# LiXirong/pytorch-r2d2

Hardware: AMD Instinct MI355X
Metric: learner_steps_per_sec (higher is better)
Workload: dtype fp32; 1 GPU; model=r2d2-qnet (reference model.py: conv32x3 + LSTM256 + dueling, 6 actions), preset=atari57, global_batch=64, per_gpu_batch=64, seq_len=80, burn_in=40, n_step=5, target_mode=fixed, matmul=bf16x3 split (fp32 accumulate, fp32 state/storage), replay_rows_per_gpu=999936, parallelism=dp1, hip_graph=True, hoisted_step=True, graph_chunk=8

## Files before the change

csrc/kernels/torso.hip:

```cpp
#include "../common.h"

template <int CIN_, int H_, int W_>
struct TGeo {
  static constexpr int CIN = CIN_, H = H_, W = W_;
  static constexpr int IN_BYTES = CIN * H * W;
  static constexpr int IN_CHUNKS = IN_BYTES / 16;
  static constexpr int NT = 512;
  static constexpr int PF = (IN_CHUNKS + 319) / 320;
  static constexpr int H1 = (H - 8) / 4 + 1, W1 = (W - 8) / 4 + 1;
  static constexpr int H2 = (H1 - 4) / 2 + 1, W2 = (W1 - 4) / 2 + 1;
  static constexpr int H3 = H2 - 2, W3 = W2 - 2;
  static constexpr int P1 = H1 * W1, P2 = H2 * W2, P3 = H3 * W3;
  static constexpr int OUT = 32 * P3;
  static constexpr int H4 = H / 4, W4 = W / 4;
  static constexpr int K1S = 4 * CIN;
  static constexpr int ACTS = 40;
  static constexpr int W2S = 512 + 8;
  static constexpr int W3S = 288 + 8;
  static constexpr int S2DS = 16 * CIN + 8;
  static constexpr int OFF_IN = 0;
  static constexpr int OFF_A1 = OFF_IN + H4 * W4 * S2DS * 2;
  static constexpr int A1_BYTES = ((P1 + 3) / 4) * 256;
  static constexpr int OFF_A2 = OFF_A1 + A1_BYTES;
  static constexpr int OFF_W2 = OFF_A2 + P2 * ACTS * 2;
  static constexpr int OFF_W3 = OFF_W2 + 32 * W2S * 2;
  static constexpr int OFF_B23 = OFF_W3 + 32 * W3S * 2;
  static constexpr int LDS_BYTES = OFF_B23 + 64 * 4;
  static_assert(H % 4 == 0 && W % 4 == 0 && IN_BYTES % 16 == 0, "geometry");
  static_assert((P1 + 31) / 32 == 13 && (P2 + 31) / 32 == 3 && (P3 + 31) / 32 == 2, "tile deal");
  static_assert(OFF_A1 % 16 == 0 && LDS_BYTES <= 160 * 1024, "LDS");
};
using GeoAtari = TGeo<4, 84, 84>;
using GeoDmlab = TGeo<3, 72, 96>;
// ... 3 lines not shown

__device__ __forceinline__ int tf_a1_off(int P, int c) {
  return ((P >> 2) << 8) + (((((P & 3) << 2) | c) ^ ((P >> 2) & 15)) << 4);
}

__device__ __forceinline__ int tf_chunk(int t) { return (t & ~63) | ((t * 25) & 63); }

template <class Gm>
__device__ __forceinline__ void torso_store_chunk(bf16* s2d, int c, const u32x4& v) {
  constexpr int RD = Gm::W / 4, PD = Gm::H * RD;
  int d = 4 * c;
  int ci = d / PD, r = d - ci * PD;
  int y = r / RD, X = r - y * RD;
#pragma unroll
  for (int e = 0; e < 4; ++e) {
    const uint32_t w = v[e];
    bf16x4 o;
    o[0] = (bf16)(float)(w & 0xff);
    o[1] = (bf16)(float)((w >> 8) & 0xff);
    o[2] = (bf16)(float)((w >> 16) & 0xff);
    o[3] = (bf16)(float)(w >> 24);
    *(bf16x4*)(s2d + ((y >> 2) * Gm::W4 + X) * Gm::S2DS + ci * 16 + (y & 3) * 4) = o;
    if (++X == RD) {
      X = 0;
      if (++y == Gm::H) { y = 0; ++ci; }
    }
  }
}

__constant__ int c_t1_begin[8] = {0, 2, 4, 5, 5, 7, 9, 11};
__constant__ int c_t1_count[8] = {2, 2, 1, 0, 2, 2, 2, 2};

#define TF_MAX_JOBS 4
struct TFJob {
  const int* rows;
  const bf16* w1; const float* b1;
  const bf16* w2; const float* b2;
  const bf16* w3; const float* b3;
  bf16* out; bf16* save1; bf16* save2;
  int n, wbegin, wcount, pad_;
};
struct TFArgs {
  const uint8_t* frames;
  TFJob job[TF_MAX_JOBS];
  int njobs, reserve_xcds, reserve_slots, pad_;
  long long* dbg;
  long long row_bytes;
};

__device__ __forceinline__ int tf_worker(int reserve_xcds, int reserve_slots) {
  const int b = blockIdx.x;
  if (reserve_slots <= 0) return b;
  const int x = b & 7, s = b >> 3, keep = 32 - reserve_slots;
  if (s < keep) return b;
  if (x < reserve_xcds) return -1;
  return keep * 8 + (s - keep) * (8 - reserve_xcds) + (x - reserve_xcds);
}

template <class Gm>
__global__ __launch_bounds__(512) void torso_fwd_kernel(const TFArgs args) {
  constexpr int NT = Gm::NT, PF = Gm::PF, IN_CHUNKS = Gm::IN_CHUNKS;
  constexpr int P1 = Gm::P1, P2 = Gm::P2, P3 = Gm::P3, ACTS = Gm::ACTS;
  constexpr int W2S = Gm::W2S, W3S = Gm::W3S, S2DS = Gm::S2DS, K1S = Gm::K1S;
  extern __shared__ __attribute__((aligned(16))) uint8_t lds[];
  bf16* in_bf = (bf16*)(lds + Gm::OFF_IN);
  bf16* act1 = (bf16*)(lds + Gm::OFF_A1);
  bf16* act2 = (bf16*)(lds + Gm::OFF_A2);
  bf16* lw2 = (bf16*)(lds + Gm::OFF_W2);
  bf16* lw3 = (bf16*)(lds + Gm::OFF_W3);
  const int tid = threadIdx.x, wave = tid >> 6, lane = tid & 63;
  const int half = lane >> 5, l32 = lane & 31;
  const int wk = tf_worker(args.reserve_xcds, args.reserve_slots);
  if (wk < 0) return;
// ... 103 lines not shown
        const int khkw = s >> 1, kh = khkw / 3, kw = khkw % 3;
        return *(const bf16x8*)(bbase + (kh * Gm::W2 + kw) * ACTS + (s & 1) * 16);
      });
      if (p < P3) {
        bf16* o = out + (size_t)fprev * Gm::OUT + p;
#pragma unroll
        for (int r = 0; r < 16; ++r) {
          const int co = (r & 3) + 8 * (r >> 2) + 4 * half;
          o[co * P3] = (bf16)fmaxf(acc[r] + lb23[32 + co], 0.f);
        }
      }
    }
    TF_TRACE(1);
    lds_sync();
    TF_TRACE(2);
    if (!have) break;

    if (conv2_wave) {
      const int p = wave * 32 + l32;
      const int pc = p < P2 ? p : P2 - 1;
      const int oy = pc / Gm::W2, ox = pc % Gm::W2;
      const bf16* abase = lw2 + l32 * W2S + half * 8;
      int oz;
      asm volatile("v_mov_b32 %0, 0" : "=v"(oz));
      const int P0 = (2 * oy) * Gm::W1 + 2 * ox + oz;
      const uint8_t* a1b = (const uint8_t*)act1;
      f32x16 acc = {};
      mfma_pipe<32, 3>(acc, [&](int s) { return *(const bf16x8*)(abase + s * 16); }, [&](int s) {
        const int khkw = s >> 1, kh = khkw >> 2, kw = khkw & 3;
        return *(const bf16x8*)(a1b + tf_a1_off(P0 + kh * Gm::W1 + kw, (s & 1) * 2 + half));
      });
      TF_TRACE(4);
      if (p < P2) {
        bf16* d2 = save2 ? save2 + ((size_t)f * P2 + p) * 32 : nullptr;
#pragma unroll
        for (int g = 0; g < 4; ++g) {
          bf16x4 v;
#pragma unroll
          for (int e = 0; e < 4; ++e) {
            const int co = 4 * half + 8 * g + e;
            v[e] = (bf16)fmaxf(acc[4 * g + e] + lb23[co], 0.f);
          }
          *(bf16x4*)(act2 + p * ACTS + 8 * g + 4 * half) = v;
          if (d2) *(bf16x4*)(d2 + 8 * g + 4 * half) = v;
        }
      }
    } else if (save1 != nullptr) {
      const int t5 = tid - 192;
      bf16* d1 = save1 + (size_t)f * P1 * 32;
      for (int i = t5; i < P1 * 4; i += 320) {
        const int row = i >> 4, pcv = (i & 15) ^ (row & 15);
        const int px = row * 4 + (pcv >> 2), q = pcv & 3;
        if (px < P1) *(bf16x8*)(d1 + px * 32 + q * 8) = *(const bf16x8*)((const uint8_t*)act1 + i * 16);
      }
    }
    TF_TRACE(5);
    if (fn < n_frames && wave >= 3) {
#pragma unroll
      for (int q = 0; q < PF; ++q) {
        const int c = tf_chunk(tid - 192 + q * 320);
        if (c < IN_CHUNKS) torso_store_chunk<Gm>(in_bf, c, pf[q]);
      }
    }
    TF_TRACE(6);
    lds_sync();
    TF_TRACE(3);
    fprev = f;
    f = fn;
    row_nx = row_nn;
    ++it_dbg;
  }
}

__global__ void frames_to_bf16_kernel(const uint8_t* __restrict__ frames, const int* __restrict__ rows,
                                      int n_frames, bf16* __restrict__ out) {
  const int f = blockIdx.y;
  const size_t row = rows ? (size_t)ld_uniform_i32(rows, f) : (size_t)f;
  const uint8_t* src = frames + row * torso::IN_BYTES;
  bf16* dst = out + (size_t)f * torso::IN_BYTES;
  for (int c = blockIdx.x * blockDim.x + threadIdx.x; c < torso::IN_BYTES / 8;
       c += gridDim.x * blockDim.x) {
    const u32x2 v = ((const u32x2*)src)[c];
// ... 138 lines not shown


static long long* g_tf_dbg = nullptr;
extern "C" int r2_torso_fwd_set_debug(long long* p) { g_tf_dbg = p; return 0; }

template <class Gm>
static void tf_launch(const TFArgs& a, int grid, hipStream_t s) {
  static bool attr_set = false;
  if (!attr_set) {
    hipFuncSetAttribute((const void*)torso_fwd_kernel<Gm>, hipFuncAttributeMaxDynamicSharedMemorySize,
                        Gm::LDS_BYTES);
    attr_set = true;
  }
  hipLaunchKernelGGL(torso_fwd_kernel<Gm>, dim3(grid), dim3(Gm::NT), Gm::LDS_BYTES, s, a);
}

extern "C" int r2_torso_fwd_geom(const uint8_t* frames, long long row_bytes, const int64_t* jobs,
                                 int njobs, int grid, int reserve_xcds, int reserve_slots, int cin,
                                 int h, int w, void* stream) {
  if (njobs < 1 || njobs > TF_MAX_JOBS) return -1;
  if (reserve_slots < 0 || reserve_slots >= 32 || reserve_xcds < 0 || reserve_xcds > 8) return -2;
  const bool atari = cin == 4 && h == 84 && w == 84, dm = cin == 3 && h == 72 && w == 96;
  if (!atari && !dm) return -6;
  const long long fb = (long long)cin * h * w;
  if (row_bytes <= 0) row_bytes = fb;
  if (row_bytes < fb || row_bytes % 16) return -7;
  TFArgs a{};
  a.frames = frames;
  a.row_bytes = row_bytes;
  a.njobs = 0;
  a.reserve_xcds = reserve_xcds;
  a.reserve_slots = reserve_slots;
  a.dbg = g_tf_dbg;
  int64_t total = 0;
  for (int i = 0; i < njobs; ++i) total += jobs[12 * i + 1] > 0 ? jobs[12 * i + 1] : 0;
  if (total <= 0) return 0;
  if (reserve_slots > 0) grid = 256;
  if (grid <= 0) grid = 256;
  const int nw = reserve_slots > 0 ? (32 - reserve_slots) * 8 + reserve_slots * (8 - reserve_xcds)
                                   : grid;
  int wb = 0;
  int64_t seen = 0;
  for (int i = 0; i < njobs; ++i) {
    const int64_t* p = jobs + 12 * i;
    if (p[1] <= 0) continue;
    seen += p[1];
    int end = (int)((seen * nw + total - 1) / total);
    if (end > nw) end = nw;
    int cnt = end - wb;
    if (cnt < 1) cnt = 1;
    if (cnt > p[1]) cnt = (int)p[1];
    TFJob& J = a.job[a.njobs++];
    J.rows = (const int*)p[0]; J.n = (int)p[1];
    J.w1 = (const bf16*)p[2]; J.b1 = (const float*)p[3];
    J.w2 = (const bf16*)p[4]; J.b2 = (const float*)p[5];
    J.w3 = (const bf16*)p[6]; J.b3 = (const float*)p[7];
    J.out = (bf16*)p[8]; J.save1 = (bf16*)p[9]; J.save2 = (bf16*)p[10];
    J.wbegin = wb; J.wcount = cnt; J.pad_ = 0;
    wb += cnt;
  }
  if (wb > nw) return -3;
  if (reserve_slots <= 0 && grid > wb) grid = wb;
  if (atari) tf_launch<GeoAtari>(a, grid, (hipStream_t)stream);
  else tf_launch<GeoDmlab>(a, grid, (hipStream_t)stream);
  R2_CHECK_LAUNCH();
  return 0;
}

extern "C" int r2_torso_fwd_multi(const uint8_t* frames, const int64_t* jobs, int njobs,
                                  int grid, int reserve_xcds, int reserve_slots, void* stream) {
  return r2_torso_fwd_geom(frames, 0, jobs, njobs, grid, reserve_xcds, reserve_slots, 4, 84, 84,
                           stream);
}

extern "C" int r2_torso_fwd(const uint8_t* frames, const int* rows, int n_frames,
                            const bf16* w1, const float* b1, const bf16* w2, const float* b2,
                            const bf16* w3, const float* b3, bf16* out, bf16* save1, bf16* save2,
                            int max_blocks, void* stream) {
  if (n_frames <= 0) return 0;
  const int64_t job[12] = {(int64_t)rows, n_frames, (int64_t)w1, (int64_t)b1, (int64_t)w2,
                           (int64_t)b2, (int64_t)w3, (int64_t)b3, (int64_t)out, (int64_t)save1,
                           (int64_t)save2, 0};
  return r2_torso_fwd_multi(frames, job, 1, max_blocks, 0, 0, stream);
}

extern "C" int r2_frames_to_bf16(const uint8_t* frames, const int* rows, int n_frames, bf16* out,
                                 void* stream) {
  if (n_frames <= 0) return 0;
  hipLaunchKernelGGL(frames_to_bf16_kernel, dim3(4, n_frames), dim3(256), 0, (hipStream_t)stream,
                     frames, rows, n_frames, out);
  R2_CHECK_LAUNCH();
// ... 3 lines not shown
```

csrc/kernels/torso_sp.hip:

```cpp
#include <type_traits>

#include "../common.h"
#include "../split.h"

namespace tsp {
constexpr int IN_BYTES = 4 * 84 * 84;
constexpr int NT = 512;
constexpr int P1 = 400, P2 = 81, P3 = 49;
}

#define TS_MAX_JOBS 4
#define TS_JOB_WORDS 20
struct TSJob {
  const int* rows;
  const bf16* w1; const bf16* w1l; const float* b1;
  const bf16* w2; const bf16* w2l; const float* b2;
  const bf16* w3; const bf16* w3l; const float* b3;
  bf16* out; bf16* out_l;
  bf16* s1; bf16* s1l;
  bf16* s2; bf16* s2l;
  unsigned* q;
  int n, wbegin, wcount, qmode;
  int pad_j[2];
};
struct TSArgs {
  const uint8_t* frames;
  TSJob job[TS_MAX_JOBS];
  int njobs, dbg;
  int dyn;
  int pad_;
  long long* trace;
};

__device__ __forceinline__ int ts_grab(const TSJob& J) {
  unsigned* q = J.q;
  if (__hip_atomic_load(q + 2, __ATOMIC_RELAXED, __HIP_MEMORY_SCOPE_AGENT) != 0u) return J.n;
  const unsigned g = __hip_atomic_fetch_add(q, 1u, __ATOMIC_RELAXED, __HIP_MEMORY_SCOPE_AGENT);
  return g < (unsigned)J.n ? (int)g : J.n;
}

__device__ __forceinline__ __amdgpu_buffer_rsrc_t ts_rsrc(const void* p, uint32_t bytes) {
  return __builtin_amdgcn_make_buffer_rsrc((void*)p, 0, bytes, 0x00020000);
}

namespace tsp2 {
using tsp::NT; using tsp::IN_BYTES; using tsp::P1; using tsp::P2; using tsp::P3;
constexpr int OFF_FR = 0;
constexpr int OFF_A1H = OFF_FR + 4 * 84 * 84;
constexpr int OFF_A1L = OFF_A1H + 400 * 64;
constexpr int OFF_A2H = OFF_A1L + 400 * 64;
constexpr int OFF_A2L = OFF_A2H + 81 * 40 * 2;
constexpr int OFF_W2H = OFF_A2L + 81 * 40 * 2;
constexpr int OFF_W2L = OFF_W2H + 32 * 520 * 2;
constexpr int OFF_B = OFF_W2L + 32 * 520 * 2;
constexpr int OFF_W3T = OFF_B + 96 * 4;
constexpr int LDS_BYTES = OFF_W3T + 2 * 32 * 32 * 2;
// ... 99 lines not shown
  for (int c = 0; c < 2; ++c)
#pragma unroll
    for (int kb = 0; kb < 4; ++kb)
#pragma unroll
      for (int d = 0; d < 3; ++d) {
        const int slot = 12 * c + 3 * kb + d;
        const bf16x8 v = *(const bf16x8*)(dig + d * 8192 + (16 * c + l16) * 256 + (4 * kb + g) * 16);
        if (slot < 16) wfh[slot & 15] = v;
        else wfl[(slot - 16) & 15] = v;
      }
}

__constant__ int c_s2_begin[8] = {0, 2, 4, 4, 6, 8, 10, 11};
__constant__ int c_s2_count[8] = {2, 2, 0, 2, 2, 2, 1, 2};

template <bool QUEUE>
__global__ __launch_bounds__(512) void torso_fwd_sp2_kernel(const TSArgs args) {
  using namespace tsp2;
  extern __shared__ __attribute__((aligned(16))) uint8_t lds[];
  uint8_t* fr = lds + OFF_FR;
  uint8_t* a1h = lds + OFF_A1H;
  uint8_t* a1l = lds + OFF_A1L;
  bf16* a2h = (bf16*)(lds + OFF_A2H);
  bf16* a2l = (bf16*)(lds + OFF_A2L);
  bf16* w2h = (bf16*)(lds + OFF_W2H);
  bf16* w2l = (bf16*)(lds + OFF_W2L);
  float* lb = (float*)(lds + OFF_B);
  uint8_t* w3t = lds + OFF_W3T;
  const int tid = threadIdx.x, wave = tid >> 6, lane = tid & 63;
  const int half = lane >> 5, l32 = lane & 31;
  const int wk = blockIdx.x;
  int ji = 0, wbeg = 0, wcnt = 0;
  if (args.dyn) {
    int ne[TS_MAX_JOBS];
    int64_t nw_[TS_MAX_JOBS];
    int64_t total = 0;
#pragma unroll
    for (int i = 0; i < TS_MAX_JOBS; ++i) {
      const TSJob& Ji = args.job[i];
      int v = i < args.njobs ? Ji.n : 0;
      if (i < args.njobs && Ji.qmode == 2)
        v -= (int)min(__hip_atomic_load(Ji.q, __ATOMIC_RELAXED, __HIP_MEMORY_SCOPE_AGENT), (unsigned)Ji.n);
      ne[i] = v;
      nw_[i] = v > 0 ? v : 0;
      total += nw_[i];
    }
    const int nw = gridDim.x;
    int wb = 0, left = 0;
#pragma unroll
    for (int i = 0; i < TS_MAX_JOBS; ++i) left += ne[i] > 0;
    int64_t seen = 0;
    ji = -1;
#pragma unroll
    for (int i = 0; i < TS_MAX_JOBS; ++i) {
      if (ne[i] <= 0) continue;
      --left;
      seen += nw_[i];
      int end = (int)((seen * nw + total - 1) / total);
      end = min(end, nw - left);
      const int cnt = min(max(end - wb, 1), ne[i]);
      if (wk >= wb && wk < wb + cnt) {
        ji = i;
        wbeg = wb;
        wcnt = cnt;
      }
      wb += cnt;
    }
    if (ji < 0) return;
  } else {
#pragma unroll
    for (int i = 1; i < TS_MAX_JOBS; ++i)
      if (i < args.njobs && wk >= args.job[i].wbegin) ji = i;
    wbeg = args.job[ji].wbegin;
    wcnt = args.job[ji].wcount;
  }
  const TSJob& J = args.job[ji];
  const int stride = wcnt;
  if (wk - wbeg >= stride) return;
  const int n_frames = J.n;
  const bool qjob = QUEUE && J.q != nullptr && J.qmode == 1;
  if (!QUEUE && J.q != nullptr && J.qmode == 1) return;
  __shared__ int s_q[4];
  int f = wk - wbeg;
  if (J.q != nullptr && J.qmode == 2)
    f += (int)min(__hip_atomic_load(J.q, __ATOMIC_RELAXED, __HIP_MEMORY_SCOPE_AGENT), (unsigned)n_frames);
  int row_f = 0, row_q1 = 0, f_q1 = 0;
  if (qjob) {
    if (tid == 0) {
      const int g0 = ts_grab(J);
      const int g1 = g0 < n_frames ? ts_grab(J) : n_frames;
      s_q[0] = g0;
      s_q[1] = g1;
      s_q[2] = g0 < n_frames ? (J.rows ? J.rows[g0] : g0) : 0;
      s_q[3] = g1 < n_frames ? (J.rows ? J.rows[g1] : g1) : 0;
    }
    __syncthreads();
    f = __builtin_amdgcn_readfirstlane(s_q[0]);
    f_q1 = __builtin_amdgcn_readfirstlane(s_q[1]);
    row_f = __builtin_amdgcn_readfirstlane(s_q[2]);
// ... 228 lines not shown
        c2_pixel(wave, l32, oy, ox, dup);
        const int p = oy * 9 + ox;
        const bf16* ah = w2h + l32 * 520 + half * 8;
        const bf16* al = w2l + l32 * 520 + half * 8;
        int vb[4];
#pragma unroll
        for (int q = 0; q < 4; ++q) {
          const int by = oy + (q >> 1), bx = ox + (q & 1);
          vb[q] = (((by * 10 + bx) << 8) | ((a1_m(by, bx) ^ half) << 4)) + oz;
        }
        constexpr int D = 2;
        bf16x8 rah[D], ral[D], rbh[D], rbl[D];
        auto ld = [&](int s, bf16x8& xah, bf16x8& xal, bf16x8& xbh, bf16x8& xbl) {
          const int khkw = s >> 1, kh = khkw >> 2, kw = khkw & 3;
          const int q = 2 * (kh >> 1) + (kw >> 1), sub = 2 * (kh & 1) + (kw & 1);
          int ob;
          asm volatile("v_xor_b32 %0, %1, %2" : "=v"(ob) : "i"(((sub << 2) | ((s & 1) << 1)) << 4), "v"(vb[q]));
          xah = *(const bf16x8*)(ah + s * 16);
          xal = *(const bf16x8*)(al + s * 16);
          xbh = *(const bf16x8*)(a1h + ob);
          xbl = *(const bf16x8*)(a1l + ob);
        };
#pragma unroll
        for (int s = 0; s < D; ++s) ld(s, rah[s], ral[s], rbh[s], rbl[s]);
        f32x16 acc = {};
#pragma unroll
        for (int s = 0; s < 32; ++s) {
          const bf16x8 xah = rah[s % D], xal = ral[s % D], xbh = rbh[s % D], xbl = rbl[s % D];
          if (s + D < 32) ld(s + D, rah[s % D], ral[s % D], rbh[s % D], rbl[s % D]);
          __builtin_amdgcn_sched_barrier(0);
          acc = mfma32_x3(xah, xal, xbh, xbl, acc);
        }
        if (!dup) {
          bf16* d2 = J.s2 ? J.s2 + ((size_t)f * P2 + p) * 32 : nullptr;
          bf16* d2l = J.s2 ? J.s2l + ((size_t)f * P2 + p) * 32 : nullptr;
#pragma unroll
          for (int g = 0; g < 4; ++g) {
            bf16x4 vh, vl;
#pragma unroll
            for (int e = 0; e < 4; ++e) {
              const int co = 4 * half + 8 * g + e;
              const float v = fmaxf(acc[4 * g + e] + lb[co], 0.f);
              vh[e] = (bf16)v;
              vl[e] = sp_lo(v);
            }
            *(bf16x4*)(a2h + p * 40 + 8 * g + 4 * half) = vh;
            *(bf16x4*)(a2l + p * 40 + 8 * g + 4 * half) = vl;
            if (d2) {
              *(bf16x4*)(d2 + 8 * g + 4 * half) = vh;
              *(bf16x4*)(d2l + 8 * g + 4 * half) = vl;
            }
          }
        }
      }
    } else {
      if (J.s1 != nullptr && !(args.dbg & 64)) {
        bf16* d1 = J.s1 + (size_t)f * P1 * 32;
        bf16* d1l = J.s1l + (size_t)f * P1 * 32;
        for (int i = tid - 192; i < P1 * 4; i += 320) {
          const int blk = i >> 4, by = blk / 10, bx = blk - 10 * by;
          const int v = (i & 15) ^ a1_m(by, bx), sub = v >> 2, c = v & 3;
          const int P = (2 * by + (sub >> 1)) * 20 + 2 * bx + (sub & 1);
          *(bf16x8*)(d1 + P * 32 + c * 8) = *(const bf16x8*)(a1h + i * 16);
          *(bf16x8*)(d1l + P * 32 + c * 8) = *(const bf16x8*)(a1l + i * 16);
        }
      }
    }
    TS2_STAMP(3);
    lds_sync();
    TS2_STAMP(4);
    ++it_dbg;
    if (qjob) {
      fnn = __builtin_amdgcn_readfirstlane(s_q[0]);
      row_nn = __builtin_amdgcn_readfirstlane(s_q[1]);
    }
    fprev = f;
    f = fn;
    f_nx = fnn;
    row_nx = row_nn;
  }
}

static int g_tsp_dbg = 0;
static long long* g_tsp_trace = nullptr;
extern "C" int r2_torso_sp_trace(long long* p) { g_tsp_trace = p; return 0; }
extern "C" int r2_torso_sp_debug(int bits) { g_tsp_dbg = bits; return 0; }

extern "C" int r2_torso_fwd_sp_multi(const uint8_t* frames, const int64_t* jobs, int njobs,
                                     int grid, void* stream) {
  if (njobs < 1 || njobs > TS_MAX_JOBS) return -1;
  TSArgs a{};
  a.frames = frames;
  a.dbg = g_tsp_dbg;
  a.trace = g_tsp_trace;
  auto wt = [&](const int64_t* p) -> int64_t { return p[1] > 0 ? p[1] : 0; };
  int64_t total = 0;
  for (int i = 0; i < njobs; ++i) total += wt(jobs + TS_JOB_WORDS * i);
  if (total <= 0) return 0;
  if (grid <= 0) grid = 256;
  const int nw = grid;
  int wb = 0;
  int64_t seen = 0;
  for (int i = 0; i < njobs; ++i) {
    const int64_t* p = jobs + TS_JOB_WORDS * i;
    if (p[1] <= 0) continue;
    seen += wt(p);
    int end = (int)((seen * nw + total - 1) / total);
    if (end > nw) end = nw;
    int cnt = end - wb;
    if (cnt < 1) cnt = 1;
    if (cnt > p[1]) cnt = (int)p[1];
    TSJob& J = a.job[a.njobs++];
    J.rows = (const int*)p[0]; J.n = (int)p[1];
    J.w1 = (const bf16*)p[2]; J.w1l = (const bf16*)p[3]; J.b1 = (const float*)p[4];
    J.w2 = (const bf16*)p[5]; J.w2l = (const bf16*)p[6]; J.b2 = (const float*)p[7];
    J.w3 = (const bf16*)p[8]; J.w3l = (const bf16*)p[9]; J.b3 = (const float*)p[10];
    J.out = (bf16*)p[11]; J.out_l = (bf16*)p[12];
    J.s1 = (bf16*)p[13]; J.s1l = (bf16*)p[14]; J.s2 = (bf16*)p[15]; J.s2l = (bf16*)p[16];
    J.q = (unsigned*)p[17];
    J.qmode = J.q ? (int)p[18] : 0;
    if (!J.w1l || !J.w2l || !J.w3l || !J.out_l || (J.s1 && !J.s1l) || (J.s2 && !J.s2l)) return -4;
    if (J.q && (J.s1 || J.s2 || (J.qmode != 1 && J.qmode != 2))) return -5;
    if (J.qmode == 2) a.dyn = 1;
    J.wbegin = wb; J.wcount = cnt;
    wb += cnt;
  }
  if (wb > nw) return -3;
  if (grid > wb && !a.dyn) grid = wb;
  if (a.dyn && grid < a.njobs) return -3;
  bool queue = false;
  for (int i = 0; i < a.njobs; ++i) queue = queue || a.job[i].qmode == 1;
  static bool attr2 = false;
  if (!attr2) {
    hipFuncSetAttribute((const void*)torso_fwd_sp2_kernel<false>, hipFuncAttributeMaxDynamicSharedMemorySize,
                        tsp2::LDS_BYTES_I8);
    hipFuncSetAttribute((const void*)torso_fwd_sp2_kernel<true>, hipFuncAttributeMaxDynamicSharedMemorySize,
                        tsp2::LDS_BYTES_I8);
    attr2 = true;
  }
  if (queue)
    hipLaunchKernelGGL(torso_fwd_sp2_kernel<true>, dim3(grid), dim3(tsp::NT), tsp2::LDS_BYTES_I8,
                       (hipStream_t)stream, a);
  else
    hipLaunchKernelGGL(torso_fwd_sp2_kernel<false>, dim3(grid), dim3(tsp::NT), tsp2::LDS_BYTES_I8,
                       (hipStream_t)stream, a);
  R2_CHECK_LAUNCH();
  return 0;
}

namespace tbs {
constexpr int NT = 512;
constexpr int P1 = 400, P2 = 81, P3 = 49;
constexpr int IN_BYTES = 4 * 84 * 84;
constexpr int IN_CHUNKS = IN_BYTES / 16;
constexpr int R = 0;
constexpr int R_A1L = P1 * 32 * 2;
constexpr int R_A2 = 2 * P1 * 32 * 2;
constexpr int R_BYTES = IN_BYTES * 2;
constexpr int G3P = R + R_BYTES;
constexpr int G3PL = G3P + 121 * 32 * 2;
constexpr int G2P = G3PL + 121 * 32 * 2;
constexpr int G2PL = G2P + 122 * 32 * 2;
constexpr int G1H = G2PL + 122 * 32 * 2;
constexpr int G1L = G1H + 406 * 32 * 2;
constexpr int W2ST = G1H, W2PL = 4 * 32 * 128 * 2;
constexpr int TBL2 = W2ST + 2 * W2PL;
constexpr int LDS = TBL2 + 12 * 64 * 8;
constexpr int W3S = 304, W3PL = 19 * 1024;
static_assert(32 * W3S * 2 <= W3PL, "W3 plane");
constexpr int G2_TRASH = 121, G1_TRASH = 400;
constexpr int PF1 = (P1 * 4 + NT - 1) / NT;
constexpr int PFF = (IN_CHUNKS + NT - 1) / NT;
constexpr int SLAB = 32 * 256 + 32 * 512 + 32 * 288 + 96;
constexpr int OFF_W2 = 32 * 256, OFF_W3 = OFF_W2 + 32 * 512, OFF_B = OFF_W3 + 32 * 288;
static_assert(R_A2 + P2 * 32 * 2 <= R_BYTES, "R");
static_assert(LDS <= 160 * 1024 && G1L + 406 * 32 * 2 <= TBL2, "LDS");
}

struct TBSArgs {
  const uint8_t* frames;
// ... 545 lines not shown
```

pytorch_r2d2_amd/engine/learner_engine.py:

```python
from __future__ import annotations

import ctypes
from typing import Dict, List, Optional

import numpy as np
import torch

from ..config import R2D2Config
from ..models.qnet import QNet
from ..ops._lib import check, kernels, ptr, stream_handle
from ..ops.gemm import G5_CFGS, Gemm, gemm, gemm_group, gemm_sp, gemm_sp_ws_bytes, group_ws_bytes
from ..models.qnet import torso_dims
from ..ops.torso_lib import (fused_torso_fwd_geom, fused_torso_supported, gather_frames_nhwc,
                             torso_backward_library_sp, torso_forward_library,
                             torso_forward_library_sp, torso_fwd_fused)
from .layout import ParamLayout, UNITS
from .replay_hbm import HBMReplay


def _graph_upload(g) -> None:
    import os
    try:
        exec_h = int(g.raw_cuda_graph_exec())
        lib = ctypes.CDLL(os.path.join(os.path.dirname(torch.__file__), "lib", "libamdhip64.so"))
# ... 559 lines not shown
                    check(rc, "lstm_fwd_tag")
                    return
            check(k.r2_lstm_fwd_persist(arr.ctypes.data, len(chains), self.B, T, self.layout.H,
                                        ptr(self.ctr), ptr(self.err), stream_handle()),
                  "lstm_fwd_persist")
        else:
            check(k.r2_lstm_fwd(arr.ctypes.data, len(chains), self.B, T, self.layout.H, t_begin,
                                stream_handle()), "lstm_fwd")

    def _heads(self, jobs, lo=None, duel: bool = True):
        if self.sp:
            probs = [Gemm(h, pk["head1"].t(), zb, a_lo=hl, b_lo=pkl["head1"].t())
                     for (pk, h, zb, _, _), (pkl, hl) in zip(jobs, lo)]
            if self.cfg.learner.sp_gemm == "fused":
                self._gemm_sp("heads", probs, splits=[0] * len(probs), cfg=-1)
            else:
                gemm(*probs)
            zs = [zb for _, _, zb, _, _ in jobs]
        else:
            gemm(*[Gemm(h, pk["head1"].t(), zb) for pk, h, zb, _, _ in jobs])
            zs = [zb for _, _, zb, _, _ in jobs]
        self._zs = zs
        if duel:
            self._duel_fwd(jobs, zs)

    def _duel_fwd(self, jobs, zs):
        self._djobs = np.asarray([[ptr(z), ptr(pk["head_b1"]), ptr(pk["head_w2"]), ptr(pk["head_b2"]),
                                   ptr(q), ptr(zr), h.shape[0]]
                                  for (pk, h, _, q, zr), z in zip(jobs, zs)], dtype=np.int64)
        fn = kernels().r2_dueling_fwd_multi_f32 if self.sp else kernels().r2_dueling_fwd_multi
        check(fn(self._djobs.ctypes.data, len(jobs), self.layout.A, self.layout.HD, stream_handle()),
              "dueling_fwd")

    def _torso_job(self, pk, rows, out, save_at=None):
        B = self.B
        s1 = s2 = 0
        if save_at is not None:
            P1 = self.act1.shape[1] * self.act1.shape[2]
            P2 = self.act2.shape[1] * self.act2.shape[2]
            s1 = self.act1.data_ptr() + save_at * B * P1 * 2
            s2 = self.act2.data_ptr() + save_at * B * P2 * 2
        return [ptr(rows), rows.numel(), ptr(pk["conv1"]), ptr(pk["b1"]), ptr(pk["conv2"]),
                ptr(pk["b2"]), ptr(pk["conv3"]), ptr(pk["b3"]), ptr(out), s1, s2, 0]

    def _torso_job_sp(self, pk, pkl, rows, out, out_lo, save_at=None, qmode: int = 0):
        B = self.B
        s = [0, 0, 0, 0]
        if save_at is not None:
            r0, r1 = save_at * B, save_at * B + rows.numel()
            s = [ptr(self.act1[r0:r1]), ptr(self.act1_lo[r0:r1]), ptr(self.act2[r0:r1]),
                 ptr(self.act2_lo[r0:r1])]
        q = [ptr(self.tq), qmode, 0] if qmode else [0, 0, 0]
        return [ptr(rows), rows.numel(), ptr(pk["conv1"]), ptr(pkl["conv1"]), ptr(pk["b1"]),
                ptr(pk["conv2"]), ptr(pkl["conv2"]), ptr(pk["b2"]), ptr(pk["conv3"]),
                ptr(pkl["conv3"]), ptr(pk["b3"]), ptr(out), ptr(out_lo)] + s + q

    def _forward_loss(self, _presampled: bool = False):
        if not _presampled:
            self._sample()
        if self.dp_global:
            self._gather_dp()
        self._forward_rest()

    def _sample(self, set_idx: Optional[int] = None, qreset=None):
        B, Tn = self.B, self.Tn
        rp = self.replay
        if qreset is None and self.hoist:
            qreset = self.tq
        S, states = self._sample_dst(self._cur if set_idx is None else set_idx)
        rp.sample_batch(B, S["starts"], S["probs"], S["rows"], Tn, states, h_f32=self.sp,
                        qreset=qreset)
        if self.cfg.learner.zero_stored_state:
            for _, _, h, c in states:
                h.zero_()
                c.zero_()
        if self.dp_global:
            root = rp.tree[int(rp.tree_offs[-1]): int(rp.tree_offs[-1]) + 1]
            if self.device.type == "cuda":
                check(kernels().r2_dp_local_stats(ptr(root), ptr(rp.n_valid), ptr(self.probs), B,
                                                  ptr(self.dp_send), stream_handle()), "dp_local_stats")
            else:
                from ..parallel.sharded_replay import local_stats
                local_stats(root, rp.n_valid, self.probs, out=self.dp_send)

    def _sample_dst(self, i: int):
        rp, n = self.replay, self.n
        S = self._sets[i]
        h0, c0 = S["h0"], S["c0"]
        st_off = {"on": 0, "tg": 0 if self.mode == "shifted" else n, "nx": n}
        states = [(rp.hs_cs, 0, h0["on"], c0["on"]),
                  (rp.target_hs_cs, st_off["tg"], h0["tg"], c0["tg"])]
        if self.mode == "fixed":
            states.append((rp.hs_cs, n, h0["nx"], c0["nx"]))
        return S, states

    def _gather_dp(self):
        from ..parallel.sharded_replay import gather_stats
        gather_stats(self.dp_send, self.world, self.pg, out=self.dp_recv, force=self.dp)

    def _forward_rest(self, tail: bool = True):
        k = kernels()
        s = stream_handle()
        B, T, Tn, Lb, Ll, n = self.B, self.T, self.Tn, self.Lb, self.Ll, self.n
        L, rp, lc = self.layout, self.replay, self.cfg.learner
        H, A = L.H, L.A
        pk, pt = self.pk, self.pk_t
        rows = self.rows
        if self.sp_lib:
            env, mc = self.cfg.env, self.cfg.model
            torso_forward_library_sp(rp.frames, rows, L, self.master, env, mc, self.X_on,
                                     self.X_on_lo, self.act1, self.act2, save_lo=Lb * B)
            torso_forward_library_sp(rp.frames, rows[self.t_lo_tg * B:], L, self.target, env, mc,
                                     self.X_tg, self.X_tg_lo)
        elif self.sp:
            pkl, ptl = self.pk_lo, self.pk_t_lo
            Xo, Xol, Xt, Xtl = self.X_on, self.X_on_lo, self.X_tg, self.X_tg_lo
            jobs = [self._torso_job_sp(pk, pkl, rows[: Lb * B], Xo[: Lb * B], Xol[: Lb * B]),
                    self._torso_job_sp(pk, pkl, rows[Lb * B: T * B], Xo[Lb * B: T * B],
                                       Xol[Lb * B: T * B], save_at=0),
                    self._torso_job_sp(pk, pkl, rows[T * B:], Xo[T * B:], Xol[T * B:]),
                    self._torso_job_sp(pt, ptl, rows[self.t_lo_tg * B:], Xt, Xtl,
                                       qmode=2 if self.hoist else 0)]
            jobs = [j for j in jobs if j[1] > 0]
            self._tjobs = np.asarray(jobs, dtype=np.int64)
            check(k.r2_torso_fwd_sp_multi(ptr(rp.frames), self._tjobs.ctypes.data, len(jobs),
                                          self.n_cus, s), "torso_fwd_sp_multi")
        elif self.fwd_geom is not None:
            jobs = [self._torso_job(pk, rows[: Lb * B], self.X_on[: Lb * B]),
                    self._torso_job(pk, rows[Lb * B: T * B], self.X_on[Lb * B: T * B], save_at=0),
                    self._torso_job(pk, rows[T * B:], self.X_on[T * B:]),
                    self._torso_job(pt, rows[self.t_lo_tg * B:], self.X_tg)]
            jobs = [j for j in jobs if j[1] > 0]
            self._tjobs = np.asarray(jobs, dtype=np.int64)
            torso_fwd_fused(rp.frames, self._tjobs, self.fwd_geom, self.n_cus, s)
        else:
            torso_forward_library(rp.frames, rows, L, self.master, self.cfg.env, self.cfg.model,
                                  self.X_on, self.act1, self.act2, save_lo=Lb * B)
            torso_forward_library(rp.frames, rows[self.t_lo_tg * B:], L, self.target, self.cfg.env,
                                  self.cfg.model, self.X_tg)
        if self.sp:
            xp_on, xp_tg = self.xp_on, self.xp_tg
            self._gemm_sp("xproj", [
                Gemm(self.X_on, pk["w_ih"].t(), xp_on, bias=self.lstm_b, a_lo=self.X_on_lo,
                     b_lo=self.pk_lo["w_ih"].t()),
                Gemm(self.X_tg, pt["w_ih"].t(), xp_tg, bias=self.lstm_b_t, a_lo=self.X_tg_lo,
                     b_lo=self.pk_t_lo["w_ih"].t())], splits=[0, 0])
        else:
            xp_on, xp_tg = self.xp_on, self.xp_tg
            gemm(Gemm(self.X_on, pk["w_ih"].t(), xp_on, bias=self.lstm_b),
                 Gemm(self.X_tg, pt["w_ih"].t(), xp_tg, bias=self.lstm_b_t))
        self._xp = (xp_on, xp_tg)
        G = L.G
        hl = self.hseq_lo
        pkl, ptl = self.pk_lo, self.pk_t_lo
        on = self._chain_desc(xp_on, pk, self.h0["on"], self.c0["on"], self.hseq["on"],
                              self.cseq["on"], self.gates, Lb, pkl, hl.get("on"))
        tg = self._chain_desc(xp_tg, pt, self.h0["tg"], self.c0["tg"], self.hseq["tg"], self.cseq["tg"],
                              None, 0, ptl, hl.get("tg"))
        if self.mode == "shifted":
            self._lstm([on, tg], self.Tc)
        elif self.mode == "fixed":
            nx = self._chain_desc(xp_on[n * B:], pk, self.h0["nx"], self.c0["nx"], self.hseq["nx"],
                                  self.cseq["nx"], None, 0, pkl, hl.get("nx"))
# ... 783 lines not shown
```

pytorch_r2d2_amd/ops/_lib.py:

```python
from __future__ import annotations

import ctypes
import os
import threading
from pathlib import Path

import torch

_PKG = Path(__file__).resolve().parent.parent
_SO = _PKG / "_r2d2_kernels.so"
_lock = threading.Lock()
_lib = None

P = ctypes.c_void_p
I = ctypes.c_int
I64 = ctypes.c_int64
U64 = ctypes.c_uint64
F = ctypes.c_float

_SIGS = {
    "r2_abi_version": [],
    "r2_set_num_cus": [I],
    "r2_set_xcd_cus": [P],
    "r2_dp_local_stats": [P, P, P, I, P, P],
# ... 5 lines not shown
    "r2_torso_fwd_multi": [P, P, I, I, I, I, P],
    "r2_torso_fwd_geom": [P, I64, P, I, I, I, I, I, I, I, P],
    "r2_frames_to_bf16": [P, P, I, P, P],
    "r2_frames_to_bf16_nhwc": [P, P, I, P, P],
    "r2_frames_gather_nhwc": [P, I64, P, I, I, I, F, P, P],
    "r2_bias_relu_nhwc_bf16": [P, P, I, I64, P],
    "r2_relu_mask_bf16": [P, P, P, I64, P],
    "r2_dueling_fwd": [P, P, P, P, P, P, I, I, I, P],
    "r2_dueling_bwd": [P, P, P, P, P, I, I, I, P],
    "r2_td_loss": [P, P, P, P, P, P, P, P, P, P, P, P, P, P, I, I, I, I, I, F, I, F, F, F, F, P, P, P,
                   P],
    "r2_td_duel": [P, P, P, P, P, P, P, P, P, P, P, P, P, P, I, I, I, I, I, F, I, F, F, F, F, P, P,
                   P, P, P, P, I, P, P, P],
    "r2_td_duel_dh": [P, P, P, P, P, P, P, P, P, P, P, P, P, P, I, I, I, I, I, F, I, F, F, F, F, P, P,
                      P, P, P, P, I, P, P, P, P, P, I, P],
    "r2_dueling_fwd_multi_f32": [P, I, I, I, P],
    "r2_lstm_fwd_tag_sp": [P, I, I, I, I, P, P, P, P],
    "r2_lstm_bwd_tag_sp": [P, P, P, P, P, P, P, P, I, I, I, I, P, P, P, P, P, P, P, P],
    "r2_lstm_bwd_tag_sp_hg": [P, P, P, P, P, P, P, P, I, I, I, I, P, P, P, P, P, P, P,
                              P, P, P, P, P, P, P, I, I, I, P, P, P],
    "r2_tree_sample": [P, P, P, I, I, U64, P, P, P, P],
    "r2_tree_rebuild": [P, P, P, I, P],
    "r2_tree_update": [P, P, P, I, P, P, I, P],
    "r2_tree_update_fused": [P, P, P, I, P, P, I, P, P, P],
    "r2_tree_update_fused_reset": [P, P, P, I, P, P, I, P, P],
    "r2_seqprio_refresh": [P, I, P, P, P, I, I, I, I, F, P, P, I, P],
    "r2_mark_starts": [P, P, I, P, P, P, I, I, F, P, P, P, I, P],
    "r2_hoist_guard": [P, I, P, P, P, I, I, I, I, P, I, P, P],
    "r2_make_rows": [P, I, I, I, I, P, P],
    "r2_sample_batch": [P, P, P, I, I, U64, P, P, P, P, I, I, I, I, P, P, P, P, P],
    "r2_sample_batch_f32h": [P, P, P, I, I, U64, P, P, P, P, I, I, I, I, P, P, P, P, P],
    "r2_sample_batch_q": [P, P, P, I, I, U64, P, P, P, P, I, I, I, I, P, P, P, P, I, P, P],
    "r2_torso_fwd_sp_multi": [P, P, I, I, P],
    "r2_torso_sp_debug": [I],
    "r2_td_duel_set_done": [P],
    "r2_prio_tail_set_wait": [P],
    "r2_torso_sp_trace": [P],
    "r2_torso_bwd_sp_trace": [P],
    "r2_torso_bwd_sp_debug": [I],
    "r2_torso_bwd_sp": [P, P, I, P, P, P, P, P, P, P, P, P, P, P, P, I, P, P, P, P],
    "r2_torso_grad_reduce": [P, I, P, P, P, P],
    "r2_gather_state": [P, P, I, I, I, I, P, P, P, P],
    "r2_step_end": [P, P, P],
    "r2_rmsprop_centered": [P, P, P, P, I64, F, F, F, F, P, F, P],
    "r2_rmsprop_pack": [P, P, P, P, I64, F, F, F, F, P, F, P, P, P, I64, P, P, I64, P],
    "r2_rmsprop_pack_slab": [P, P, P, P, I64, F, F, F, F, P, P, P, I64, P, P, I64, P, I, I, P, P, I64, P],
    "r2_adam": [P, P, P, P, I64, F, F, F, F, F, P, P, F, P],
    "r2_sumsq": [P, I64, P, P],
    "r2_pack_bf16": [P, P, P, I64, P],
    "r2_gather_f32": [P, P, P, I64, P],
    "r2_copy_if_due": [P, P, I64, P, I64, P],
    "r2_noop_chain": [P, I, I, P],
    "r2_torso_bwd": [P, P, I, P, P, P, P, P, P, P, I, P, P, P, P],
    "r2_torso_bwd_slab_floats": [],
    "r2_torso_bwd_geom": [P, I64, P, I, P, P, P, P, P, P, P, I, P, P, P, I, I, I, P],
    "r2_torso_bwd_slab_floats_geom": [I, I, I],
    "r2_gemm": [P, I, P],
    "r2_gemm_set_version": [I],
    "r2_gemm_group": [P, P, I, P, I64, P, I, P],
    "r2_dueling_fwd_multi": [P, I, I, I, P],
    "r2_actor_pre": [P, P],
    "r2_actor_post": [P, P],
    "r2_actor_tail": [P, P],
    "r2_actor_args_bytes": [],
    "r2_pack_step": [P, P, I64, P, P, P, I64, P, P, P, I64, I64, I64, P, P, I64, P, I64, I64, P],
    "r2_pack_split": [P, P, P, I64, I64, P],
# ... 119 lines not shown
```

Baseline: 1127 learner steps/s of the whole job, one step = a 64 x 80-step sequence batch (= optimizer steps/s x 1 ranks; global batch 64).

## Merge online torso jobs with a save window and balance work-group deal

The three online torso jobs (burn-in, trained span, tail) become one job whose activation saving is limited to a frame window [save_lo, save_hi). A new shared torso_deal routine assigns work-groups to jobs by minimising the maximum frames per worker, falling back to the old proportional split. It runs on host and on device for the dynamic qmode path. The goal is fewer job boundaries and less load imbalance across work-groups, at the cost of a per-frame window check and more complex dealing logic in each block.

Result: no change. 1131 learner steps/s of the whole job, one step = a 64 x 80-step sequence batch (= optimizer steps/s x 1 ranks; global batch 64) (median of 2 runs) (+0.3%).

```diff
diff --git a/csrc/kernels/torso.hip b/csrc/kernels/torso.hip
--- a/csrc/kernels/torso.hip
+++ b/csrc/kernels/torso.hip
@@ -1,4 +1,5 @@
 #include "../common.h"
+#include "../torso_deal.h"
 
 template <int CIN_, int H_, int W_>
 struct TGeo {
@@ -68,13 +69,15 @@
 __constant__ int c_t1_count[8] = {2, 2, 1, 0, 2, 2, 2, 2};
 
 #define TF_MAX_JOBS 4
+static_assert(TF_MAX_JOBS == TORSO_DEAL_JOBS, "torso_deal.h deals TF_MAX_JOBS jobs");
 struct TFJob {
   const int* rows;
   const bf16* w1; const float* b1;
   const bf16* w2; const float* b2;
   const bf16* w3; const float* b3;
   bf16* out; bf16* save1; bf16* save2;
-  int n, wbegin, wcount, pad_;
+  int n, wbegin, wcount, save_lo;
+  int save_hi, pad_;
 };
 struct TFArgs {
   const uint8_t* frames;
@@ -244,7 +247,8 @@
       });
       TF_TRACE(4);
       if (p < P2) {
-        bf16* d2 = save2 ? save2 + ((size_t)f * P2 + p) * 32 : nullptr;
+        bf16* d2 = save2 && f >= J.save_lo && f < J.save_hi
+                       ? save2 + ((size_t)(f - J.save_lo) * P2 + p) * 32 : nullptr;
 #pragma unroll
         for (int g = 0; g < 4; ++g) {
           bf16x4 v;
@@ -257,9 +261,9 @@
           if (d2) *(bf16x4*)(d2 + 8 * g + 4 * half) = v;
         }
       }
-    } else if (save1 != nullptr) {
+    } else if (save1 != nullptr && f >= J.save_lo && f < J.save_hi) {
       const int t5 = tid - 192;
-      bf16* d1 = save1 + (size_t)f * P1 * 32;
+      bf16* d1 = save1 + (size_t)(f - J.save_lo) * P1 * 32;
       for (int i = t5; i < P1 * 4; i += 320) {
         const int row = i >> 4, pcv = (i & 15) ^ (row & 15);
         const int px = row * 4 + (pcv >> 2), q = pcv & 3;
@@ -464,24 +468,23 @@
   a.reserve_xcds = reserve_xcds;
   a.reserve_slots = reserve_slots;
   a.dbg = g_tf_dbg;
-  int64_t total = 0;
-  for (int i = 0; i < njobs; ++i) total += jobs[12 * i + 1] > 0 ? jobs[12 * i + 1] : 0;
-  if (total <= 0) return 0;
+  int nfr[TF_MAX_JOBS] = {}, wc[TF_MAX_JOBS];
+  for (int i = 0; i < njobs; ++i) {
+    const int64_t n = jobs[12 * i + 1];
+    if (n > INT32_MAX) return -1;
+    nfr[i] = n > 0 ? (int)n : 0;
+  }
   if (reserve_slots > 0) grid = 256;
   if (grid <= 0) grid = 256;
   const int nw = reserve_slots > 0 ? (32 - reserve_slots) * 8 + reserve_slots * (8 - reserve_xcds)
                                    : grid;
+  const int worst = torso_deal(nfr, nw, wc);
+  if (worst <= 0) return worst;
   int wb = 0;
-  int64_t seen = 0;
   for (int i = 0; i < njobs; ++i) {
     const int64_t* p = jobs + 12 * i;
     if (p[1] <= 0) continue;
-    seen += p[1];
-    int end = (int)((seen * nw + total - 1) / total);
-    if (end > nw) end = nw;
-    int cnt = end - wb;
-    if (cnt < 1) cnt = 1;
-    if (cnt > p[1]) cnt = (int)p[1];
+    const int cnt = wc[i];
     TFJob& J = a.job[a.njobs++];
     J.rows = (const int*)p[0]; J.n = (int)p[1];
     J.w1 = (const bf16*)p[2]; J.b1 = (const float*)p[3];
@@ -489,6 +492,10 @@
     J.w3 = (const bf16*)p[6]; J.b3 = (const float*)p[7];
     J.out = (bf16*)p[8]; J.save1 = (bf16*)p[9]; J.save2 = (bf16*)p[10];
     J.wbegin = wb; J.wcount = cnt; J.pad_ = 0;
+    J.save_lo = (int)(p[11] & 0xffffffffll);
+    J.save_hi = (int)(p[11] >> 32);
+    if (J.save_lo == 0 && J.save_hi == 0) J.save_hi = J.n;
+    if (J.save_lo < 0 || J.save_hi < J.save_lo || J.save_hi > J.n) return -8;
     wb += cnt;
   }
   if (wb > nw) return -3;
diff --git a/csrc/kernels/torso_sp.hip b/csrc/kernels/torso_sp.hip
--- a/csrc/kernels/torso_sp.hip
+++ b/csrc/kernels/torso_sp.hip
@@ -2,6 +2,7 @@
 
 #include "../common.h"
 #include "../split.h"
+#include "../torso_deal.h"
 
 namespace tsp {
 constexpr int IN_BYTES = 4 * 84 * 84;
@@ -11,6 +12,7 @@
 
 #define TS_MAX_JOBS 4
 #define TS_JOB_WORDS 20
+static_assert(TS_MAX_JOBS == TORSO_DEAL_JOBS, "torso_deal.h deals TS_MAX_JOBS jobs");
 struct TSJob {
   const int* rows;
   const bf16* w1; const bf16* w1l; const float* b1;
@@ -21,7 +23,7 @@
   bf16* s2; bf16* s2l;
   unsigned* q;
   int n, wbegin, wcount, qmode;
-  int pad_j[2];
+  int save_lo, save_hi;
 };
 struct TSArgs {
   const uint8_t* frames;
@@ -187,9 +189,7 @@
   const int wk = blockIdx.x;
   int ji = 0, wbeg = 0, wcnt = 0;
   if (args.dyn) {
-    int ne[TS_MAX_JOBS];
-    int64_t nw_[TS_MAX_JOBS];
-    int64_t total = 0;
+    int ne[TS_MAX_JOBS], wc[TS_MAX_JOBS];
 #pragma unroll
     for (int i = 0; i < TS_MAX_JOBS; ++i) {
       const TSJob& Ji = args.job[i];
@@ -197,29 +197,18 @@
       if (i < args.njobs && Ji.qmode == 2)
         v -= (int)min(__hip_atomic_load(Ji.q, __ATOMIC_RELAXED, __HIP_MEMORY_SCOPE_AGENT), (unsigned)Ji.n);
       ne[i] = v;
-      nw_[i] = v > 0 ? v : 0;
-      total += nw_[i];
-    }
-    const int nw = gridDim.x;
-    int wb = 0, left = 0;
-#pragma unroll
-    for (int i = 0; i < TS_MAX_JOBS; ++i) left += ne[i] > 0;
-    int64_t seen = 0;
+    }
+    if (torso_deal(ne, (int)gridDim.x, wc) <= 0) return;
+    int wb = 0;
     ji = -1;
 #pragma unroll
     for (int i = 0; i < TS_MAX_JOBS; ++i) {
-      if (ne[i] <= 0) continue;
-      --left;
-      seen += nw_[i];
-      int end = (int)((seen * nw + total - 1) / total);
-      end = min(end, nw - left);
-      const int cnt = min(max(end - wb, 1), ne[i]);
-      if (wk >= wb && wk < wb + cnt) {
+      if (wk >= wb && wk < wb + wc[i]) {
         ji = i;
         wbeg = wb;
-        wcnt = cnt;
-      }
-      wb += cnt;
+        wcnt = wc[i];
+      }
+      wb += wc[i];
     }
     if (ji < 0) return;
   } else {
@@ -514,8 +503,9 @@
           acc = mfma32_x3(xah, xal, xbh, xbl, acc);
         }
         if (!dup) {
-          bf16* d2 = J.s2 ? J.s2 + ((size_t)f * P2 + p) * 32 : nullptr;
-          bf16* d2l = J.s2 ? J.s2l + ((size_t)f * P2 + p) * 32 : nullptr;
+          const bool sv = J.s2 != nullptr && f >= J.save_lo && f < J.save_hi;
+          bf16* d2 = sv ? J.s2 + ((size_t)(f - J.save_lo) * P2 + p) * 32 : nullptr;
+          bf16* d2l = sv ? J.s2l + ((size_t)(f - J.save_lo) * P2 + p) * 32 : nullptr;
 #pragma unroll
           for (int g = 0; g < 4; ++g) {
             bf16x4 vh, vl;
@@ -536,9 +526,9 @@
         }
       }
     } else {
-      if (J.s1 != nullptr && !(args.dbg & 64)) {
-        bf16* d1 = J.s1 + (size_t)f * P1 * 32;
-        bf16* d1l = J.s1l + (size_t)f * P1 * 32;
+      if (J.s1 != nullptr && f >= J.save_lo && f < J.save_hi && !(args.dbg & 64)) {
+        bf16* d1 = J.s1 + (size_t)(f - J.save_lo) * P1 * 32;
+        bf16* d1l = J.s1l + (size_t)(f - J.save_lo) * P1 * 32;
         for (int i = tid - 192; i < P1 * 4; i += 320) {
           const int blk = i >> 4, by = blk / 10, bx = blk - 10 * by;
           const int v = (i & 15) ^ a1_m(by, bx), sub = v >> 2, c = v & 3;
@@ -575,23 +565,21 @@
   a.frames = frames;
   a.dbg = g_tsp_dbg;
   a.trace = g_tsp_trace;
-  auto wt = [&](const int64_t* p) -> int64_t { return p[1] > 0 ? p[1] : 0; };
-  int64_t total = 0;
-  for (int i = 0; i < njobs; ++i) total += wt(jobs + TS_JOB_WORDS * i);
-  if (total <= 0) return 0;
+  int nfr[TS_MAX_JOBS] = {}, wc[TS_MAX_JOBS];
+  for (int i = 0; i < njobs; ++i) {
+    const int64_t n = jobs[TS_JOB_WORDS * i + 1];
+    if (n > INT32_MAX) return -1;
+    nfr[i] = n > 0 ? (int)n : 0;
+  }
   if (grid <= 0) grid = 256;
   const int nw = grid;
+  const int worst = torso_deal(nfr, nw, wc);
+  if (worst <= 0) return worst;
   int wb = 0;
-  int64_t seen = 0;
   for (int i = 0; i < njobs; ++i) {
     const int64_t* p = jobs + TS_JOB_WORDS * i;
     if (p[1] <= 0) continue;
-    seen += wt(p);
-    int end = (int)((seen * nw + total - 1) / total);
-    if (end > nw) end = nw;
-    int cnt = end - wb;
-    if (cnt < 1) cnt = 1;
-    if (cnt > p[1]) cnt = (int)p[1];
+    const int cnt = wc[i];
     TSJob& J = a.job[a.njobs++];
     J.rows = (const int*)p[0]; J.n = (int)p[1];
     J.w1 = (const bf16*)p[2]; J.w1l = (const bf16*)p[3]; J.b1 = (const float*)p[4];
@@ -603,6 +591,10 @@
     J.qmode = J.q ? (int)p[18] : 0;
     if (!J.w1l || !J.w2l || !J.w3l || !J.out_l || (J.s1 && !J.s1l) || (J.s2 && !J.s2l)) return -4;
     if (J.q && (J.s1 || J.s2 || (J.qmode != 1 && J.qmode != 2))) return -5;
+    J.save_lo = (int)(p[19] & 0xffffffffll);
+    J.save_hi = (int)(p[19] >> 32);
+    if (J.save_lo == 0 && J.save_hi == 0) J.save_hi = J.n;
+    if (J.save_lo < 0 || J.save_hi < J.save_lo || J.save_hi > J.n) return -6;
     if (J.qmode == 2) a.dyn = 1;
     J.wbegin = wb; J.wcount = cnt;
     wb += cnt;
@@ -628,6 +620,15 @@
                        (hipStream_t)stream, a);
   R2_CHECK_LAUNCH();
   return 0;
+}
+
+extern "C" int r2_torso_deal(const int* n, int njobs, int grid, int* wcount) {
+  if (njobs < 1 || njobs > TORSO_DEAL_JOBS) return -1;
+  int nfr[TORSO_DEAL_JOBS] = {}, wc[TORSO_DEAL_JOBS];
+  for (int i = 0; i < njobs; ++i) nfr[i] = n[i];
+  const int worst = torso_deal(nfr, grid, wc);
+  for (int i = 0; i < njobs; ++i) wcount[i] = wc[i];
+  return worst;
 }
 
 namespace tbs {
diff --git a/csrc/torso_deal.h b/csrc/torso_deal.h
--- /dev/null
+++ b/csrc/torso_deal.h
@@ -0,0 +1,74 @@
+#pragma once
+#include <stdint.h>
+
+#define TORSO_DEAL_JOBS 4
+#define TORSO_DEAL_TRIES 64
+
+#if defined(__HIPCC__) || defined(__CUDACC__)
+#define TORSO_DEAL_HD __host__ __device__
+#else
+#define TORSO_DEAL_HD
+#endif
+
+TORSO_DEAL_HD inline int torso_deal(const int (&n)[TORSO_DEAL_JOBS], int grid,
+                                    int (&wcount)[TORSO_DEAL_JOBS]) {
+  int64_t total = 0;
+  int live = 0;
+#pragma unroll
+  for (int i = 0; i < TORSO_DEAL_JOBS; ++i) {
+    wcount[i] = 0;
+    if (n[i] > 0) {
+      total += n[i];
+      ++live;
+    }
+  }
+  if (live == 0) return 0;
+  if (grid < live) return -3;
+  const int64_t m0 = (total + grid - 1) / grid;
+  if (m0 < INT32_MAX - TORSO_DEAL_TRIES) {
+    int m = (int)m0;
+    for (int t = 0; t < TORSO_DEAL_TRIES; ++t, ++m) {
+      int used = 0;
+#pragma unroll
+      for (int i = 0; i < TORSO_DEAL_JOBS; ++i)
+        if (n[i] > 0) used += (n[i] - 1) / m + 1;
+      if (used > grid) continue;
+#pragma unroll
+      for (int i = 0; i < TORSO_DEAL_JOBS; ++i)
+        if (n[i] > 0) wcount[i] = (n[i] - 1) / m + 1;
+      for (int left = grid - used, t2 = 0; left > 0 && t2 < TORSO_DEAL_TRIES; --left, ++t2) {
+        int best = -1, bn = 0, bc = 1;
+#pragma unroll
+        for (int i = 0; i < TORSO_DEAL_JOBS; ++i)
+          if (n[i] > wcount[i] && (best < 0 || (int64_t)n[i] * bc > (int64_t)bn * wcount[i])) {
+            best = i;
+            bn = n[i];
+            bc = wcount[i];
+          }
+        if (best < 0) break;
+#pragma unroll
+        for (int i = 0; i < TORSO_DEAL_JOBS; ++i)
+          if (i == best) ++wcount[i];
+      }
+      return m;
+    }
+  }
+  int wb = 0, left = live, worst = 0;
+  int64_t seen = 0;
+#pragma unroll
+  for (int i = 0; i < TORSO_DEAL_JOBS; ++i) {
+    if (n[i] <= 0) continue;
+    --left;
+    seen += n[i];
+    int end = (int)((seen * grid + total - 1) / total);
+    if (end > grid - left) end = grid - left;
+    int cnt = end - wb;
+    if (cnt < 1) cnt = 1;
+    if (cnt > n[i]) cnt = n[i];
+    wcount[i] = cnt;
+    wb += cnt;
+    const int per = (n[i] - 1) / cnt + 1;
+    if (per > worst) worst = per;
+  }
+  return worst;
+}
diff --git a/pytorch_r2d2_amd/engine/learner_engine.py b/pytorch_r2d2_amd/engine/learner_engine.py
--- a/pytorch_r2d2_amd/engine/learner_engine.py
+++ b/pytorch_r2d2_amd/engine/learner_engine.py
@@ -615,25 +615,39 @@
         check(fn(self._djobs.ctypes.data, len(jobs), self.layout.A, self.layout.HD, stream_handle()),
               "dueling_fwd")
 
-    def _torso_job(self, pk, rows, out, save_at=None):
+    @staticmethod
+    def _save_window(window):
+        if window is None:
+            return 0
+        lo, hi = window
+        assert 0 <= lo < hi < 2 ** 31
+        return lo | (hi << 32)
+
+    def _torso_job(self, pk, rows, out, save_at=None, window=None):
         B = self.B
         s1 = s2 = 0
+        if window is not None and save_at is None:
+            save_at = 0
         if save_at is not None:
             P1 = self.act1.shape[1] * self.act1.shape[2]
             P2 = self.act2.shape[1] * self.act2.shape[2]
             s1 = self.act1.data_ptr() + save_at * B * P1 * 2
             s2 = self.act2.data_ptr() + save_at * B * P2 * 2
         return [ptr(rows), rows.numel(), ptr(pk["conv1"]), ptr(pk["b1"]), ptr(pk["conv2"]),
-                ptr(pk["b2"]), ptr(pk["conv3"]), ptr(pk["b3"]), ptr(out), s1, s2, 0]
-
-    def _torso_job_sp(self, pk, pkl, rows, out, out_lo, save_at=None, qmode: int = 0):
+                ptr(pk["b2"]), ptr(pk["conv3"]), ptr(pk["b3"]), ptr(out), s1, s2,
+                self._save_window(window)]
+
+    def _torso_job_sp(self, pk, pkl, rows, out, out_lo, save_at=None, qmode: int = 0, window=None):
         B = self.B
         s = [0, 0, 0, 0]
+        if window is not None and save_at is None:
+            save_at = 0
         if save_at is not None:
-            r0, r1 = save_at * B, save_at * B + rows.numel()
+            r0 = save_at * B
+            r1 = r0 + (rows.numel() if window is None else window[1] - window[0])
             s = [ptr(self.act1[r0:r1]), ptr(self.act1_lo[r0:r1]), ptr(self.act2[r0:r1]),
                  ptr(self.act2_lo[r0:r1])]
-        q = [ptr(self.tq), qmode, 0] if qmode else [0, 0, 0]
+        q = [ptr(self.tq), qmode, 0] if qmode else [0, 0, self._save_window(window)]
         return [ptr(rows), rows.numel(), ptr(pk["conv1"]), ptr(pkl["conv1"]), ptr(pk["b1"]),
                 ptr(pk["conv2"]), ptr(pkl["conv2"]), ptr(pk["b2"]), ptr(pk["conv3"]),
                 ptr(pkl["conv3"]), ptr(pk["b3"]), ptr(out), ptr(out_lo)] + s + q
@@ -698,10 +712,7 @@
         elif self.sp:
             pkl, ptl = self.pk_lo, self.pk_t_lo
             Xo, Xol, Xt, Xtl = self.X_on, self.X_on_lo, self.X_tg, self.X_tg_lo
-            jobs = [self._torso_job_sp(pk, pkl, rows[: Lb * B], Xo[: Lb * B], Xol[: Lb * B]),
-                    self._torso_job_sp(pk, pkl, rows[Lb * B: T * B], Xo[Lb * B: T * B],
-                                       Xol[Lb * B: T * B], save_at=0),
-                    self._torso_job_sp(pk, pkl, rows[T * B:], Xo[T * B:], Xol[T * B:]),
+            jobs = [self._torso_job_sp(pk, pkl, rows, Xo, Xol, window=(Lb * B, T * B)),
                     self._torso_job_sp(pt, ptl, rows[self.t_lo_tg * B:], Xt, Xtl,
                                        qmode=2 if self.hoist else 0)]
             jobs = [j for j in jobs if j[1] > 0]
@@ -709,9 +720,7 @@
             check(k.r2_torso_fwd_sp_multi(ptr(rp.frames), self._tjobs.ctypes.data, len(jobs),
                                           self.n_cus, s), "torso_fwd_sp_multi")
         elif self.fwd_geom is not None:
-            jobs = [self._torso_job(pk, rows[: Lb * B], self.X_on[: Lb * B]),
-                    self._torso_job(pk, rows[Lb * B: T * B], self.X_on[Lb * B: T * B], save_at=0),
-                    self._torso_job(pk, rows[T * B:], self.X_on[T * B:]),
+            jobs = [self._torso_job(pk, rows, self.X_on, window=(Lb * B, T * B)),
                     self._torso_job(pt, rows[self.t_lo_tg * B:], self.X_tg)]
             jobs = [j for j in jobs if j[1] > 0]
             self._tjobs = np.asarray(jobs, dtype=np.int64)
diff --git a/pytorch_r2d2_amd/ops/_lib.py b/pytorch_r2d2_amd/ops/_lib.py
--- a/pytorch_r2d2_amd/ops/_lib.py
+++ b/pytorch_r2d2_amd/ops/_lib.py
@@ -61,6 +61,7 @@
     "r2_sample_batch_f32h": [P, P, P, I, I, U64, P, P, P, P, I, I, I, I, P, P, P, P, P],
     "r2_sample_batch_q": [P, P, P, I, I, U64, P, P, P, P, I, I, I, I, P, P, P, P, I, P, P],
     "r2_torso_fwd_sp_multi": [P, P, I, I, P],
+    "r2_torso_deal": [P, I, I, P],
     "r2_torso_sp_debug": [I],
     "r2_td_duel_set_done": [P],
     "r2_prio_tail_set_wait": [P],
```
